# vsergeev/luaradio

Hardware: AMD Instinct MI355X
Metric: MSamples/s per block (128-tap complex FIR headline) + WBFM chain end-to-end (higher is better)
Workload: dtype f32

## Files before the change

luaradio_amd/csrc/kernels_fir.h:

```cpp
#pragma once
#include "common.h"
#include "kernels_elem.h"

#ifndef LRHIP_FIR_PIPE
#define LRHIP_FIR_PIPE 2
#endif
#ifndef LRHIP_DISC_EPI_LDS
#define LRHIP_DISC_EPI_LDS 0
#endif

namespace lrhip {

typedef float f32x4 __attribute__((ext_vector_type(4)));

#ifndef LRHIP_FIR_SETPRIO
#define LRHIP_FIR_SETPRIO 0
#endif
#ifndef LRHIP_FIR_SCHED
#define LRHIP_FIR_SCHED 0
#endif
#ifndef LRHIP_FIR_XCD_MAP
#define LRHIP_FIR_XCD_MAP 0
#endif
#ifndef LRHIP_FIR_WAVES_PER_SIMD
// ... 140 lines not shown
            v1 = o.y;
        } else if (ROT) {
            float2 o = rotate_sample(make_float2(v0, v1), rot_step_fx, rot_count0 + (uint64_t)(p - (M - 1)));
            v0 = o.x;
            v1 = o.y;
        }
        int pa = G::phys(S * r);
        ldsX[pa] = v0;
        if (S == 2) ldsX[pa + 1] = v1;
    }
}

__host__ __device__ constexpr int fir_taps_zl(int D) { return 3 + 15 * D; }
__host__ __device__ constexpr int fir_taps_len(int D, int ksteps) { return ((fir_taps_zl(D) + 4 * ksteps + 3) / 4) * 4; }

template <int S, int D, int NACC, int KS, int NOUT, int TQS = 0>
__device__ __forceinline__ void mfma_tile(const float *ldsT, int tlen, int e, const float *ldsX, int ksteps, f32x4 (&acc)[NOUT][NACC])
{
    using G = FirMfmaGeom<S, D>;
    const int lane = threadIdx.x & 63, wave = threadIdx.x >> 6;
    const int col = lane & 15, kq = lane >> 4;
    const int blk_in_acc = S == 2 ? (col >> 1) : col;
    const int comp = S == 2 ? (col & 1) : 0;
    constexpr int ACC_STRIDE = (G::ROW + G::PAD) * G::BPA;
    const float *bptr = ldsX + (G::ROW + G::PAD) * ((wave * NACC) * G::BPA + blk_in_acc) + S * kq + comp;
    const float *aptr = ldsT + kq * TQS + fir_taps_zl(D) + kq - e - col * D;
#pragma unroll
    for (int o = 0; o < NOUT; o++)
#pragma unroll
        for (int a = 0; a < NACC; a++) acc[o][a] = (f32x4){0.f, 0.f, 0.f, 0.f};
    auto step = [&](const float *ap, const float *bp, int j) {
        float av[NOUT];
#pragma unroll
        for (int o = 0; o < NOUT; o++) av[o] = ap[o * tlen + 4 * j];
#pragma unroll
        for (int a = 0; a < NACC; a++) {
            float bv = bp[a * ACC_STRIDE + j * 4 * S];
#pragma unroll
            for (int o = 0; o < NOUT; o++) acc[o][a] = __builtin_amdgcn_mfma_f32_16x16x4f32(av[o], bv, acc[o][a], 0, 0, 0);
        }
    };
    if constexpr (KS > 0 && (LRHIP_FIR_PIPE == 1 || (LRHIP_FIR_PIPE == 2 && D > 1))) {
        float av[2][NOUT], bv[2][NACC];
        auto fetch = [&](int buf, int s) {
            const int g = s / G::GROUP, j = s % G::GROUP;
            const float *ap = aptr + 4 * g * G::GROUP, *bp = bptr + g * (G::ROW + G::PAD);
#pragma unroll
            for (int o = 0; o < NOUT; o++) av[buf][o] = ap[o * tlen + 4 * j];
#pragma unroll
            for (int a = 0; a < NACC; a++) bv[buf][a] = bp[a * ACC_STRIDE + j * 4 * S];
        };
        fetch(0, 0);
#pragma unroll
        for (int s = 0; s < KS; s++) {
            if (s + 1 < KS) fetch((s + 1) & 1, s + 1);
            __builtin_amdgcn_sched_barrier(0);
#pragma unroll
            for (int a = 0; a < NACC; a++)
#pragma unroll
                for (int o = 0; o < NOUT; o++) acc[o][a] = __builtin_amdgcn_mfma_f32_16x16x4f32(av[s & 1][o], bv[s & 1][a], acc[o][a], 0, 0, 0);
            __builtin_amdgcn_sched_barrier(0);
        }
    } else if constexpr (KS > 0) {
#if LRHIP_FIR_SETPRIO
        __builtin_amdgcn_s_setprio(1);
#endif
#pragma unroll
        for (int g = 0; g < (KS + G::GROUP - 1) / G::GROUP; g++)
#pragma unroll
            for (int j = 0; j < G::GROUP; j++)
// ... 14 lines not shown
}

template <int S, int D, int KS, int TQS, int NR>
__device__ __forceinline__ void mfma_load_areg(const float *ldsT, int e, float (&areg)[NR])
{
    using G = FirMfmaGeom<S, D>;
    const int lane = threadIdx.x & 63;
    const int col = lane & 15, kq = lane >> 4;
    const float *aptr = ldsT + kq * TQS + fir_taps_zl(D) + kq - e - col * D;
#pragma unroll
    for (int s = 0; s < NR; s++) areg[s] = aptr[4 * (s / G::GROUP) * G::GROUP + 4 * (s % G::GROUP)];
}
#ifndef LRHIP_MFMA_AREG_DEPTH
#define LRHIP_MFMA_AREG_DEPTH 1
#endif
template <int S, int D, int NACC, int KS, int TQS, int NR, int SPLIT = 1>
__device__ __forceinline__ void mfma_tile_areg(const float (&areg)[NR], const float *ldsT, int e, const float *ldsX, f32x4 (&acc)[1][NACC])
{
    using G = FirMfmaGeom<S, D>;
    static_assert(NR <= KS, "register-resident steps");
    const int lane = threadIdx.x & 63, wave = threadIdx.x >> 6;
    const int col = lane & 15, kq = lane >> 4;
    const int blk_in_acc = S == 2 ? (col >> 1) : col;
    const int comp = S == 2 ? (col & 1) : 0;
    constexpr int ACC_STRIDE = (G::ROW + G::PAD) * G::BPA;
    const float *bptr = ldsX + (G::ROW + G::PAD) * ((wave * NACC) * G::BPA + blk_in_acc) + S * kq + comp;
    const float *aptr = ldsT + kq * TQS + fir_taps_zl(D) + kq - e - col * D;
    f32x4 acc2[NACC];
#pragma unroll
    for (int a = 0; a < NACC; a++) acc[0][a] = acc2[a] = (f32x4){0.f, 0.f, 0.f, 0.f};
    constexpr int DEPTH = LRHIP_MFMA_AREG_DEPTH, NB = DEPTH + 1;
    float bv[NB][NACC], av[NB];
    auto fetch = [&](int buf, int s) {
        const int g = s / G::GROUP, j = s % G::GROUP;
        const float *bp = bptr + g * (G::ROW + G::PAD);
#pragma unroll
        for (int a = 0; a < NACC; a++) bv[buf][a] = bp[a * ACC_STRIDE + j * 4 * S];
        if (s >= NR) av[buf] = aptr[4 * g * G::GROUP + 4 * j];
    };
#pragma unroll
    for (int s = 0; s < DEPTH && s < KS; s++) fetch(s % NB, s);
#pragma unroll
    for (int s = 0; s < KS; s++) {
        if (s + DEPTH < KS) fetch((s + DEPTH) % NB, s + DEPTH);
        __builtin_amdgcn_sched_barrier(0);
#pragma unroll
        for (int a = 0; a < NACC; a++) {
            const float af = s < NR ? areg[s < NR ? s : 0] : av[s % NB];
            if (SPLIT == 2 && (s & 1)) acc2[a] = __builtin_amdgcn_mfma_f32_16x16x4f32(af, bv[s % NB][a], acc2[a], 0, 0, 0);
            else acc[0][a] = __builtin_amdgcn_mfma_f32_16x16x4f32(af, bv[s % NB][a], acc[0][a], 0, 0, 0);
        }
        __builtin_amdgcn_sched_barrier(0);
    }
    if (SPLIT == 2) {
#pragma unroll
        for (int a = 0; a < NACC; a++) acc[0][a] += acc2[a];
    }
}

// ... 539 lines not shown
            float *o = y + 2 * k;
            if (out_aligned && k + 3 < n_out) {
                *reinterpret_cast<float4 *>(o) = make_float4(dl[0], acc[0][a][0], dl[1], acc[0][a][1]);
                *reinterpret_cast<float4 *>(o + 4) = make_float4(dl[2], acc[0][a][2], dl[3], acc[0][a][3]);
            } else {
#pragma unroll
                for (int i = 0; i < 4; i++)
                    if (k + i < n_out) *reinterpret_cast<float2 *>(o + 2 * i) = make_float2(dl[i], acc[0][a][i]);
            }
        }
    } else {
        store_tile<S, D, NACC, NOUT>(y, tile_k0, n_out, out_aligned, acc);
    }
}

template <int S, int D, int NACC, bool ROT, int KS, int EPI = 0, bool REL = false, int NW = 4, int FMT = 0>
__global__ __launch_bounds__(64 * NW, LRHIP_FIR_WAVES_PER_SIMD) void fir_mfma_persistent_kernel(
    const float *__restrict__ hist, const float *__restrict__ x, const float *__restrict__ taps_pad, float *__restrict__ y,
    int M, long n, long n_out, long first, int e, long ntiles, int out_aligned,
    uint64_t rot_step_fx, uint64_t rot_count0, float2 *__restrict__ edge, float2 *__restrict__ prev_out, double inv_gain, float *__restrict__ hist_out, int rounds)
{
    using G = FirMfmaGeom<S, D>;
    constexpr int NT = 64 * NW;
    static_assert(NW == 4 || (NW == 1 && REL), "one-wave workgroups: relative rotator staging + discriminator epilogue only");
    constexpr int TILE_OUT = G::tile_out(NACC, NW);
    constexpr int SPAN = G::span(NACC, KS, NW);
    static_assert(FMT == 0 || (S == 2 && !REL && EPI == 0 && NW == 4), "raw records: the plain Tuner / Decimator instantiations");
    if (hist_out && blockIdx.x == 0)
        for (int i = threadIdx.x; i < (M - 1) * S; i += NT) hist_out[i] = FMT ? stream_at_raw<FMT>(hist, x, n + i / S, i % S, M, n) : stream_at<S>(hist, x, n + i / S, i % S, M, n);
    constexpr int NF4 = SPAN * S / 4;
    constexpr int UX = (NF4 + NT - 1) / NT;
    extern __shared__ __attribute__((aligned(16))) float lds[];
    constexpr int TLEN = fir_taps_len(D, KS);
    float *ldsT = lds;
    float *ldsX = lds + TLEN;
    const int tid = threadIdx.x;
// ... 50 lines not shown
                const int idx = i4_of(u), ic = idx < 0 ? 0 : idx < NF4 ? idx : NF4 - 1;
                if (FMT == RX_FMT_S16LE) praw[FMT ? u : 0] = reinterpret_cast<const uint2 *>(src0)[ic];
                else praw[FMT ? u : 0].x = reinterpret_cast<const unsigned *>(src0)[ic];
            }
        } else if (have) {
            const float4 *src = reinterpret_cast<const float4 *>(x + xlo_of(tt) * S);
#pragma unroll
            for (int u = 0; u < NPRE; u++) {
                int idx = i4_of(u);
                pre[FMT ? 0 : u] = src[idx < 0 ? 0 : idx < NF4 ? idx : NF4 - 1];
            }
        }
    };
    auto pre_of = [&](int u) -> float4 { if constexpr (FMT != 0) return rx_raw_pair<FMT>(praw[u]); else return pre[u]; };
    prefetch(t);
    for (; t < ntiles; t = tile_of(++tk)) {
        const long tile_k0 = t * (long)TILE_OUT;
        if (have) {
            const long xlo = xlo_of(t);
            if constexpr (REL) {
#pragma unroll
                for (int u = 0; u < UX; u++) {
                    const int i4 = tid + u * NT;
                    const cf a = cmul(cf{pre[u].x, pre[u].y}, rel_w[u][0]), b = cmul(cf{pre[u].z, pre[u].w}, rel_w[u][1]);
                    if (i4 < NF4) lds_put4<S, D>(ldsX, i4, make_float4(a.x, a.y, b.x, b.y));
                }
            } else if constexpr (ROT) {
#pragma unroll
                for (int v = 0; v < UB; v++) {
                    const int i40 = 4 * (tid + NT * v) - a4;
// ... 9 lines not shown
                        if (i40 + 2 >= 0 && i40 + 2 < NF4) lds_put4<S, D>(ldsX, i40 + 2, rotate_in_block<2>(pre_of(4 * v + 2), p, rot_t));
                        if (i40 + 3 < NF4) lds_put4<S, D>(ldsX, i40 + 3, rotate_in_block<3>(pre_of(4 * v + 3), p, rot_t));
                    }
                }
            } else {
#pragma unroll
                for (int u = 0; u < UX; u++) {
                    const int i4 = tid + u * NT;
                    if (i4 < NF4) lds_put4<S, D>(ldsX, i4, pre_of(u));
                }
            }
        } else {
            stage_edge<S, D, ROT, REL, NT, FMT>(ldsX, hist, x, first + tile_k0 * D - e, SPAN, M, n, rot_step_fx, rot_count0);
        }
        __syncthreads();
        prefetch(tile_of(tk + 1));
        f32x4 acc[1][NACC];
        mfma_tile<S, D, NACC, KS, 1>(ldsT, TLEN, e, ldsX, KS, acc);
        if constexpr (EPI == 0) {
            store_tile<S, D, NACC, 1>(y, tile_k0, n_out, out_aligned, acc);
        } else {
            static_assert(S == 2, "discriminator epilogue: complex stream");
#if LRHIP_DISC_EPI_LDS
            disc_epilogue_lds<D, NACC>(y, ldsX, tile_k0, n_out, acc, edge + 2 * t, prev_out, inv_gain);
#else
            cf pt = cf{1.f, 0.f};
            if constexpr (REL) pt = phasor_poly(rot_step_fx * (rot_count0 + (uint64_t)xlo_of(t)));
            const bool stream_start = REL && t == 0 && rot_count0 == 0 && first == 0 && n > 0;
            float2 o_first = make_float2(0.f, 0.f);
            if constexpr (REL) {
                if (stream_start) {
                    const float h0 = ldsT[fir_taps_zl(D) + M - 1];
                    const float2 x0 = rotate_sample(*reinterpret_cast<const float2 *>(x), rot_step_fx, (uint64_t)0);
                    o_first = make_float2(fmaf(h0, x0.x, 0.f), fmaf(h0, x0.y, 0.f));
                }
            }
            disc_epilogue<D, NACC, REL>(y, tile_k0, n_out, out_aligned, acc, edge + 2 * NW * t, prev_out, inv_gain, pt, stream_start, o_first);
#endif
        }
        __syncthreads();
    }
}

inline int fir_mfma_ksteps(int M, int D, int S, int emax_override = -1)
{
    int emax = emax_override >= 0 ? emax_override : 4 / S - 1;
    return (emax + 15 * D + M + 3) / 4;
}
inline void fir_mfma_build_taps(const float *taps_rev, int M, int D, int ksteps, std::vector<float> &out)
{
    out.assign((size_t)fir_taps_len(D, ksteps), 0.f);
    for (int j = 0; j < M; j++) out[(size_t)fir_taps_zl(D) + j] = taps_rev[j];
}

}
```

luaradio_amd/csrc/kernels_rx.h:

```cpp
#pragma once
#include "kernels_fir.h"

#ifndef LRHIP_RX_AREG
#define LRHIP_RX_AREG 40
#endif
#ifndef LRHIP_RX_SPLITK
#define LRHIP_RX_SPLITK 1
#endif

namespace lrhip {

struct RxParams {
    const float *hist;
    const float *x;
    long n;
    const float *taps_pad;
    long n_out_a, first_a;
    int e;
    long ntiles;
    uint64_t rot_step_fx, rot_count0;
    const float2 *prev_in;
    float2 *prev_out;
    double inv_gain;
    float *hist_out;
// ... 70 lines not shown
    const uint8_t *b = reinterpret_cast<const uint8_t *>(x) + 2 * xi;
    return rx_raw_sample<FMT>(b[0], b[1]);
}

#ifdef LRHIP_RX_TRACE
__device__ unsigned long long *lrhip_rx_trace;
#define RX_STAMP(i)                                                                                                                                 \
    do {                                                                                                                                            \
        if (lrhip_rx_trace && blockIdx.x < 8 && trace_tile < 64 && (threadIdx.x & 63) == 0)                                                         \
            lrhip_rx_trace[(((size_t)blockIdx.x * 4 + (threadIdx.x >> 6)) * 64 + trace_tile) * 8 + (i)] = clock64();                                  \
    } while (0)
#else
#define RX_STAMP(i) do { } while (0)
#endif

template <int FMT>
__global__ __launch_bounds__(256, LRHIP_RX_WAVES_PER_SIMD) void rx_fused_kernel(const RxParams pr)
{
    constexpr bool U8 = FMT != RX_FMT_CF32;
    constexpr int NT = 256, D = RX_D, S = 2, M = RX_M;
    constexpr int NF4 = RX_SPAN * S / 4;
    constexpr int UX = (NF4 + NT - 1) / NT;
    static_assert(2 * UX <= 64, "one lane per uniform phasor");
    extern __shared__ __attribute__((aligned(16))) float lds[];
    float *ldsT = lds, *ldsX = lds + RX_LDS_X, *P = lds + RX_LDS_P, *ldsGT = lds + RX_LDS_G, *ldsPt = lds + RX_LDS_PT, *xch = lds + RX_LDS_XCH;
    float2 *eo = reinterpret_cast<float2 *>(lds + RX_LDS_EO);
    const int tid = threadIdx.x, lane = tid & 63, wave = tid >> 6;
    const long n = pr.n;
    const float *__restrict__ x = pr.x;
    const float *__restrict__ hist = pr.hist;

    if (pr.hist_out && blockIdx.x == 0)
        for (int i = tid; i < M - 1; i += NT) {
            const cf v = rx_stream_at<FMT>(hist, x, n + i, M, n);
            pr.hist_out[2 * i] = v.x;
            pr.hist_out[2 * i + 1] = v.y;
        }
    for (int i = tid; i < RX_TLEN; i += NT) {
// ... 28 lines not shown
    auto xlo_of = [&](long tt) { return pr.first_a + tt * (long)RX_TILE * D - pr.e - (M - 1); };
    auto interior = [&](long tt) { const long lo = xlo_of(tt); return tt < tend && lo >= 0 && lo + RX_SPAN <= n; };

    cf rel_w[UX][2];
    {
        const cf pt = phasor_poly(pr.rot_step_fx * (uint64_t)(2 * tid)), pu = phasor_poly(pr.rot_step_fx * (uint64_t)(2 * NT * (lane >> 1) + (lane & 1)));
#pragma unroll
        for (int u = 0; u < UX; u++)
#pragma unroll
            for (int j = 0; j < 2; j++) rel_w[u][j] = cmul(pt, cf{__shfl(pu.x, 2 * u + j), __shfl(pu.y, 2 * u + j)});
    }

    float4 pre[U8 ? 1 : UX];
    uint2 pre8[U8 ? UX : 1];
    bool have = false;
    auto prefetch = [&](long tt) {
        have = interior(tt);
        if (U8) {
            if (have) {
                const uint8_t *src0 = reinterpret_cast<const uint8_t *>(x) + 2 * rx_raw_bytes<FMT>() * xlo_of(tt);
#pragma unroll
                for (int u = 0; u < UX; u++) {
                    const int idx = tid + NT * u, ic = idx < NF4 ? idx : NF4 - 1;
                    if (FMT == RX_FMT_S16LE) pre8[u] = reinterpret_cast<const uint2 *>(src0)[ic];
                    else pre8[u].x = reinterpret_cast<const unsigned *>(src0)[ic];
                }
            }
        } else if (have && (pr.dbg & 8)) {
#pragma unroll
            for (int u = 0; u < UX; u++) pre[u] = make_float4(0.5f, 0.25f, -0.5f, 0.125f);
        } else if (have) {
            const float4 *src = reinterpret_cast<const float4 *>(x + xlo_of(tt) * S);
#pragma unroll
            for (int u = 0; u < UX; u++) {
                const int idx = tid + NT * u;
                pre[u] = src[idx < NF4 ? idx : NF4 - 1];
            }
        }
    };
    prefetch(t);

    [[maybe_unused]] int trace_tile = 0;
    for (; t < tend; t++) {
        RX_STAMP(0);
        const bool warm = t < t0;
        const int tau = warm ? RX_TPB - 1 : (int)((t - t0) % RX_TPB);
        const long bidx = warm ? 0 : (t - t0) / RX_TPB;
        const long tile_k0 = t * (long)RX_TILE;
        if (have) {
#pragma unroll
            for (int u = 0; u < UX; u++) {
                const int i4 = tid + u * NT;
                cf s0, s1;
                if (U8) {
                    if (FMT == RX_FMT_S16LE) {
                        s0 = rx_raw_sample<FMT>(pre8[u].x & 0xffffu, pre8[u].x >> 16);
                        s1 = rx_raw_sample<FMT>(pre8[u].y & 0xffffu, pre8[u].y >> 16);
// ... 12 lines not shown
        } else if (U8) {
            using GE = FirMfmaGeom<S, D>;
            const long base = pr.first_a + tile_k0 * D - pr.e;
            for (int r = tid; r < RX_SPAN; r += NT) {
                const cf o = cmul(rx_stream_at<FMT>(hist, x, base + r, M, n), rel_window_phasor<NT>(pr.rot_step_fx, r));
                const int pa = GE::phys(S * r);
                ldsX[pa] = o.x;
                ldsX[pa + 1] = o.y;
            }
        } else {
            stage_edge<S, D, true, true, NT>(ldsX, hist, x, pr.first_a + tile_k0 * D - pr.e, RX_SPAN, M, n, pr.rot_step_fx, pr.rot_count0);
        }
        RX_STAMP(1);
        __syncthreads();
        RX_STAMP(2);
        prefetch(t + 1 < tend ? t + 1 : tend);
        RX_STAMP(3);

        f32x4 acc[1][RX_NACC];
        if (pr.dbg & 4) {
#pragma unroll
            for (int a = 0; a < RX_NACC; a++) acc[0][a] = (f32x4){ldsX[tid], ldsX[tid + 256], ldsX[tid + 512], ldsX[tid + 768]};
        }
#if LRHIP_RX_AREG
        else mfma_tile_areg<S, D, RX_NACC, RX_KS, RX_TQS, LRHIP_RX_AREG, LRHIP_RX_SPLITK>(areg, ldsT, pr.e, ldsX, acc);
#else
        else mfma_tile<S, D, RX_NACC, RX_KS, 1, RX_TQS>(ldsT, RX_TLEN, pr.e, ldsX, RX_KS, acc);
#endif

        RX_STAMP(4);
#if LRHIP_RX_NACC == 1
        {
            const int col = lane & 15, kq = lane >> 4;
            const bool odd = col & 1;
            const int src = odd ? lane - 1 : kq ? lane - 15 : col ? col + 47 : 63;
            const float a0 = acc[0][0][0], a1 = acc[0][0][1], a2 = acc[0][0][2], a3 = acc[0][0][3];
            const float recv0 = __shfl_xor(odd ? a0 : a2, 1);
            const float recv1 = __shfl_xor(odd ? a1 : a3, 1);
            const float2 o0 = odd ? make_float2(recv0, a2) : make_float2(a0, recv0);
            const float2 o1 = odd ? make_float2(recv1, a3) : make_float2(a1, recv1);
            float2 p = make_float2(__shfl(o1.x, src), __shfl(o1.y, src));
            float2 *eo_t = eo + 4 * (int)(t & 1), *eo_p = eo + 4 * (int)((t & 1) ^ 1);
            if (lane == 63) eo_t[wave] = o1;
// ... 65 lines not shown
        RX_STAMP(7);
#ifdef LRHIP_RX_TRACE
        trace_tile++;
#endif
        const bool last_tile = t == pr.ntiles - 1;
        if (tau == RX_TPB - 1 || t == tend - 1) {
            __syncthreads();
            f32x4 acct[1][1];
            acct[0][0] = (f32x4){0.f, 0.f, 0.f, 0.f};
            if (!(pr.dbg & 1) && wave < RX_AW && (!warm || wave == RX_AW - 1)) mfma_tile<1, D, 1, RX_KST, 1>(ldsGT + RX_GZ, RX_GLEN - RX_GZ, phi, P, RX_KST, acct);
            float *vrow = ldsX;
            {
                const int col = lane & 15, kq = lane >> 4;
                if (wave < RX_AW) *reinterpret_cast<float4 *>(vrow + 16 * (wave * 16 + col) + 4 * kq) = make_float4(acct[0][0][0], acct[0][0][1], acct[0][0][2], acct[0][0][3]);
            }
            __syncthreads();
            const bool scan_lane = tid < 64 * RX_AW;
            float4 v4 = scan_lane ? *reinterpret_cast<const float4 *>(vrow + 4 * tid) : make_float4(0.f, 0.f, 0.f, 0.f);
            if (warm) {
                const int kmin = (RX_TH + (RX_TPB - 1) * RX_TILE + 1 - phi + 4) / 5;
                const int k = 4 * tid;
                v4 = make_float4(k >= kmin ? v4.x : 0.f, k + 1 >= kmin ? v4.y : 0.f, k + 2 >= kmin ? v4.z : 0.f, k + 3 >= kmin ? v4.w : 0.f);
            }
            const float u0 = pr.b0 * v4.x, u1 = pr.b0 * v4.y, u2 = pr.b0 * v4.z, u3 = pr.b0 * v4.w;
            auto stepq = [&](float stv, float uv) { return fmaf(pr.na1, stv, fmaf(pr.na1_lo, stv, uv)); };
            float z = stepq(stepq(stepq(u0, u1), u2), u3);
#pragma unroll
            for (int l = 0; l < 6; l++) {
                const float prev = __shfl_up(z, 1 << l);
                if (lane >= (1 << l)) z = z + fmaf(ldsPt[(1 << l) - 1], prev, 0.f);
            }
// ... 26 lines not shown
                if (!ends_with_batch && last >= 0 && last < 4) pr.state_out[0] = last == 0 ? y0 : last == 1 ? y1 : last == 2 ? y2 : y3;
                if (ends_with_batch && tid == 0) pr.state_out[0] = C;
            }
            carry = C;
            __syncthreads();
            if (last_tile) {
                const int ev = (int)(pr.n_out_a - (t0 * RX_TILE + bidx * RX_BATCH));
                if (tid < RX_TH) pr.thist_out[tid] = P[rx_pos(ev - RX_TH + tid)];
            } else if (tid < RX_TH) {
                P[rx_pos(tid - RX_TH)] = P[rx_pos(RX_BATCH - RX_TH + tid)];
            }
        }
    }
}

}
```

luaradio_amd/csrc/stage_fir.h:

```cpp
#pragma once
#include "fir_form.h"

struct FirStage : lrhip_stage, FirShape {
    FirStage() { rel_rot = !LRHIP_DISC_EPI_LDS && getenv("LRHIP_TUNER_EXACT") == nullptr;
                 rel_nw1 = getenv("LRHIP_TUNER_NW1") != nullptr; }
    std::vector<float> taps_rev;
    std::vector<float> natural_taps() const
    {
        const int ts = taps_complex ? 2 : 1;
        std::vector<float> h((size_t)M * ts);
        for (int t = 0; t < M; t++)
            for (int c = 0; c < ts; c++) h[(size_t)t * ts + c] = taps_rev[(size_t)(M - 1 - t) * ts + c];
        return h;
    }
    DeviceBuf d_taps, d_atab, d_ctaps4;
    int mfma_blocks_per_cu = 0;
    int hist_pad = 0;
    DeviceBuf hist[2];
    int cur = 0;
    unsigned long index = 0;
    uint64_t rot_step = 0, count = 0;
    long L = 0, fill = 0;
    DeviceBuf pending, work;
    static constexpr int FFT_PART = FIR_FFT_PART;
// ... 108 lines not shown
        const unsigned esz = raw_now ? (in_fmt == RX_FMT_S16LE ? 4u : 2u) : (unsigned)(4 * SS);
        if (((uintptr_t)x % esz) != 0) return set_error("fir: fused rotator / discriminator needs a sample-aligned input pointer");
        long sample_addr = (long)((uintptr_t)x / esz);
        int q = 4 / SS;
        long v = sample_addr + (long)index - (M - 1);
        int e = (int)(((v % q) + q) % q);
        int span = G::span(NACC, ksteps, NW);
        size_t lds_floats = (size_t)fir_taps_len(DD, ksteps) + (size_t)G::phys(SS * span) + G::PAD + 8;
        size_t lds_bytes = lds_floats * sizeof(float);
        long ntiles = (n_out + TILE_OUT - 1) / TILE_OUT;
        const float *atab = (const float *)d_atab.p;
        const float *h = (const float *)hist[cur].p + hist_pad;
        int out_aligned = ((uintptr_t)y % 16) == 0;
        uint64_t rs = rot ? rot_step : 0, rc = rot ? count : 0;
        if constexpr (KS > 0) {
            auto launch = [&](auto kern) -> int {
                if ((mfma_blocks_per_cu = prepared_blocks(kern, lds_bytes, 64 * NW)) < 0) return -1;
                long slots = (long)ctx().num_cus * mfma_blocks_per_cu;
                const int rounds = ntiles > slots && fir_knobs().fir_rounds > 0 ? fir_knobs().fir_rounds : 0;
                unsigned grid = rounds > 0 ? (unsigned)((ntiles + rounds - 1) / rounds) : (unsigned)(ntiles < slots ? ntiles : slots);
                if (post_disc && edge.reserve((size_t)ntiles * 2 * NW * sizeof(float2))) return -1;
                float *ho = M > 1 ? (float *)hist[cur ^ 1].p + hist_pad : nullptr;
                hipLaunchKernelGGL(kern, dim3(grid), dim3(64 * NW), lds_bytes, ctx().stream, h, x, atab, y, M, n, n_out, (long)index, e,
                                   ntiles, out_aligned, rs, rc, (float2 *)edge.p, post_disc ? (float2 *)disc_prev.p + (disc_cur ^ 1) : nullptr, 1.0 / disc_gain, ho, rounds);
                hist_in_kernel = ho != nullptr;
                return 0;
            };
            int rc2;
            if constexpr (SS == 2 && (DD == 4 || DD == 8 || DD == 10)) {
                if (!(post_disc && rot)) return set_error("internal: decimation %d has a persistent kernel for tuner + discriminator only", DD);
            }
            if constexpr (SS == 2 && (DD == 1 || DD == 5 || DD == 4 || DD == 8 || DD == 10)) {
                if (post_disc) {
                    if constexpr (DD == 4 || DD == 8 || DD == 10)
                        rc2 = rel_rot ? launch(fir_mfma_persistent_kernel<2, DD, NACC, true, KS, 1, true>) : launch(fir_mfma_persistent_kernel<2, DD, NACC, true, KS, 1, false>);
                    else if constexpr (NW == 1) rc2 = launch(fir_mfma_persistent_kernel<2, DD, NACC, true, KS, 1, true, 1>);
                    else if constexpr (LRHIP_DISC_EPI_LDS) rc2 = rot ? launch(fir_mfma_persistent_kernel<2, DD, NACC, true, KS, 1>) : launch(fir_mfma_persistent_kernel<2, DD, NACC, false, KS, 1>);
                    else rc2 = !rot ? launch(fir_mfma_persistent_kernel<2, DD, NACC, false, KS, 1>)
                             : rel_rot ? launch(fir_mfma_persistent_kernel<2, DD, NACC, true, KS, 1, true>) : launch(fir_mfma_persistent_kernel<2, DD, NACC, true, KS, 1, false>);
                    if (rc2) return rc2;
                    LR_LAUNCH_CHECK();
                    float2 *dp = (float2 *)disc_prev.p;
                    constexpr int FIX_UNIT = LRHIP_DISC_EPI_LDS ? TILE_OUT : TILE_OUT / NW;
                    const long nunits = LRHIP_DISC_EPI_LDS ? ntiles : NW * ntiles;
                    if (defer_fixup && (FIX_UNIT & (FIX_UNIT - 1)) == 0 && FIX_UNIT >= 256) {
                        fix_ready = true;
                        fix_nunits = nunits; fix_unit = FIX_UNIT;
                        fix_prev_ptr = (const float2 *)(dp + disc_cur);
                        fix_shift = 0;
                        while ((1 << fix_shift) < FIX_UNIT) fix_shift++;
                    } else {
                        hipLaunchKernelGGL(fir_disc_fixup_kernel, dim3((unsigned)((nunits + 255) / 256)), dim3(256), 0, ctx().stream, (const float2 *)edge.p,
                                           nunits, FIX_UNIT, y, n_out, (const float2 *)(dp + disc_cur), 1.0 / disc_gain);
                        LR_LAUNCH_CHECK();
                    }
                    disc_cur ^= 1;
                    return 0;
                }
            }
            if (post_disc) return set_error("internal: discriminator epilogue without a persistent kernel variant");
            if constexpr (SS == 2 && DD == 5 && KS == 51 && NW == 4) {
                if (raw_now) {
                    if (rot)
                        rc2 = in_fmt == RX_FMT_U8 ? launch(fir_mfma_persistent_kernel<2, DD, NACC, true, KS, 0, false, 4, RX_FMT_U8>)
                            : in_fmt == RX_FMT_S8 ? launch(fir_mfma_persistent_kernel<2, DD, NACC, true, KS, 0, false, 4, RX_FMT_S8>)
                                                  : launch(fir_mfma_persistent_kernel<2, DD, NACC, true, KS, 0, false, 4, RX_FMT_S16LE>);
                    else
                        rc2 = in_fmt == RX_FMT_U8 ? launch(fir_mfma_persistent_kernel<2, DD, NACC, false, KS, 0, false, 4, RX_FMT_U8>)
                            : in_fmt == RX_FMT_S8 ? launch(fir_mfma_persistent_kernel<2, DD, NACC, false, KS, 0, false, 4, RX_FMT_S8>)
                                                  : launch(fir_mfma_persistent_kernel<2, DD, NACC, false, KS, 0, false, 4, RX_FMT_S16LE>);
                    if (rc2) return rc2;
                    LR_LAUNCH_CHECK();
                    return 0;
                }
            }
            if (raw_now) return set_error("internal: raw records reached a kernel without a record instantiation");
            if constexpr (DD == 4 || DD == 8 || DD == 10) return set_error("internal: no plain persistent kernel at decimation %d", DD);
            else {
                if constexpr (SS == 2) rc2 = rot ? launch(fir_mfma_persistent_kernel<2, DD, NACC, true, KS>) : launch(fir_mfma_persistent_kernel<2, DD, NACC, false, KS>);
                else rc2 = rot ? set_error("rotator fusion needs complex input") : launch(fir_mfma_persistent_kernel<1, DD, NACC, false, KS>);
                if (rc2) return rc2;
            }
        } else {
            if (post_disc) return set_error("internal: discriminator epilogue without a persistent kernel variant");
            auto launch = [&](auto kern) -> int {
                if (prepare_kernel(kern, lds_bytes, nullptr)) return -1;
                hipLaunchKernelGGL(kern, dim3((unsigned)ntiles), dim3(256), lds_bytes, ctx().stream, h, x, atab, y, M, n, n_out, (long)index, e,
                                   ksteps, out_aligned, rs, rc);
                return 0;
            };
            int rc2;
            if constexpr (SS == 2) rc2 = rot ? launch(fir_mfma_kernel<2, DD, NACC, true, 1>) : launch(fir_mfma_kernel<2, DD, NACC, false, 1>);
            else rc2 = rot ? set_error("rotator fusion needs complex input") : launch(fir_mfma_kernel<1, DD, NACC, false, 1>);
            if (rc2) return rc2;
        }
// ... 921 lines not shown
```

luaradio_amd/csrc/stage_rx.h:

```cpp
#pragma once

struct RxStage : lrhip_stage {
    std::unique_ptr<FirStage> A, B;
    DeviceBuf mid;
    DeviceBuf d_ptab4;
    int blocks_per_cu = 0, blocks_per_cu8 = 0;
    int in_fmt = RX_FMT_CF32;
    bool in_u8 = false;
    lrhip_stage *fmt = nullptr;
    DeviceBuf converted;
    bool single_launch = true;
    int last_form = 0;

    const char *kind() const override { return "fm-receiver"; }
    bool direct_io_ok() const override { return true; }
    unsigned long max_output(unsigned long n) const override { return B->max_output(A->max_output(n)); }
    int reset() override { return (A->reset() || B->reset()) ? -1 : 0; }
    int seek(unsigned long long n0, unsigned long long *n0_out) override
    {
        unsigned long long m = 0;
        if (A->seek(n0, &m) || B->seek(m, n0_out)) return -1;
        return 0;
    }
    long memory() const override
// ... 59 lines not shown
            if (m < 0) return m;
            return run_cf32(converted.p, n_in, out_dev, cap, one, n_out_a, n_out_b, false);
        }
        return run_cf32(in_dev, n_in, out_dev, cap, one, n_out_a, n_out_b, in_u8);
    }

    long run_cf32(const void *in_dev, unsigned long n_in, void *out_dev, unsigned long cap, bool one, long n_out_a, long n_out_b, bool u8)
    {
        const long n = (long)n_in;
        if (!one || (!u8 && ((uintptr_t)in_dev % 8) != 0)) return run_two(in_dev, n_in, out_dev, cap);
        if ((unsigned long)n_out_b > cap) return set_error("fm-receiver: output capacity %lu < %ld", cap, n_out_b);
        const float *x = (const float *)in_dev;
        const size_t lds_bytes = (size_t)RX_LDS_FLOATS * sizeof(float);
        int &bpc = u8 ? blocks_per_cu8 : blocks_per_cu;
        const int fmt_k = u8 ? in_fmt : RX_FMT_CF32;
        auto with_kernel = [&](auto fn) -> int {
            switch (fmt_k) {
                case RX_FMT_U8: return fn(rx_fused_kernel<RX_FMT_U8>);
                case RX_FMT_S8: return fn(rx_fused_kernel<RX_FMT_S8>);
                case RX_FMT_S16LE: return fn(rx_fused_kernel<RX_FMT_S16LE>);
                default: return fn(rx_fused_kernel<RX_FMT_CF32>);
            }
        };
        if (!bpc) {
            const int rc0 = with_kernel([&](auto kern) -> int {
                LR_HIP(hipFuncSetAttribute((const void *)kern, hipFuncAttributeMaxDynamicSharedMemorySize, (int)lds_bytes));
                int nb = 0;
                LR_HIP(hipOccupancyMaxActiveBlocksPerMultiprocessor(&nb, kern, 256, lds_bytes));
                bpc = nb < 1 ? 1 : nb;
                return 0;
            });
            if (rc0) return rc0;
        }
        RxParams pr;
        memset(&pr, 0, sizeof(pr));
        pr.hist = (const float *)A->hist[A->cur].p; pr.x = x; pr.n = n; pr.taps_pad = (const float *)A->d_atab.p;
        pr.n_out_a = n_out_a; pr.first_a = (long)A->index;
        const long v = (long)((uintptr_t)x / (u8 ? (in_fmt == RX_FMT_S16LE ? 4 : 2) : 8)) + (long)A->index - (RX_M - 1);
        pr.e = (int)(((v % 2) + 2) % 2);
        pr.ntiles = (n_out_a + RX_TILE - 1) / RX_TILE;
// ... 12 lines not shown
        if (env_wgs > 0) wgs = (long)ctx().num_cus * env_wgs;
        const long most = (pr.ntiles + 7) / 8;
        if (wgs < 1 || wgs > most) wgs = most;
        pr.dbg = ablation_bits("LRHIP_RX_DBG");
        const unsigned grid = (unsigned)wgs;
#ifdef LRHIP_RX_TRACE
        static unsigned long long *trace = nullptr;
        static long trace_launches = 0;
        const size_t trace_n = (size_t)8 * 4 * 64 * 8;
        if (!trace) {
            LR_HIP(hipMalloc(&trace, trace_n * 8));
            LR_HIP(hipMemcpyToSymbol(HIP_SYMBOL(lrhip_rx_trace), &trace, sizeof(trace)));
        }
        if (++trace_launches == 12) LR_HIP(hipMemsetAsync(trace, 0, trace_n * 8, ctx().stream));
#endif
        (void)with_kernel([&](auto kern) -> int { hipLaunchKernelGGL(kern, dim3(grid), dim3(256), lds_bytes, ctx().stream, pr); return 0; });
        LR_LAUNCH_CHECK();
#ifdef LRHIP_RX_TRACE
        if (trace_launches == 12) {
            LR_HIP(hipStreamSynchronize(ctx().stream));
            std::vector<unsigned long long> tr(trace_n);
            LR_HIP(hipMemcpy(tr.data(), trace, trace_n * 8, hipMemcpyDeviceToHost));
            static const char *names[8] = {"stage", "barrierA", "prefetch", "mfma", "exchange", "barrierB", "disc", "tail"};
            for (int w = 0; w < 4; w++) {
                double sum[8] = {0, 0, 0, 0, 0, 0, 0, 0}, tile = 0;
                int cnt = 0;
                for (int b = 0; b < 8; b++)
                    for (int t = 2; t < 62; t++) {
                        const unsigned long long *s = &tr[(((size_t)b * 4 + w) * 64 + t) * 8], *nx = s + 8;
                        if (!s[0] || !s[7] || !nx[0]) continue;
                        for (int i = 0; i < 7; i++) sum[i] += (double)(s[i + 1] - s[i]);
// ... 23 lines not shown
```

Measured before the change: 315,500.

## Spread next-tile global prefetch across MFMA steps via hook in pipelined loop

Instead of issuing all next-tile input prefetch loads in one burst before the MFMA tile loop, the loads are spread across the k-steps of the software-pipelined MFMA loop through a per-step hook. They use wave-uniform base pointers with clamped per-lane offsets so addresses are always in bounds. The goal is to overlap global memory traffic with matrix math and smooth out issue pressure. Burst-kernel variants are kept for short inputs and debug modes, which doubles the kernel instantiations. An optional wave-level fence can replace one __syncthreads in the audio path, but only behind a macro.

Result: no change. 315,100 (-0.2%).

```diff
diff --git a/luaradio_amd/csrc/kernels_fir.h b/luaradio_amd/csrc/kernels_fir.h
--- a/luaradio_amd/csrc/kernels_fir.h
+++ b/luaradio_amd/csrc/kernels_fir.h
@@ -1,4 +1,5 @@
 #pragma once
+#include <type_traits>
 #include "common.h"
 #include "kernels_elem.h"
 
@@ -178,9 +179,47 @@
 __host__ __device__ constexpr int fir_taps_zl(int D) { return 3 + 15 * D; }
 __host__ __device__ constexpr int fir_taps_len(int D, int ksteps) { return ((fir_taps_zl(D) + 4 * ksteps + 3) / 4) * 4; }
 
-template <int S, int D, int NACC, int KS, int NOUT, int TQS = 0>
-__device__ __forceinline__ void mfma_tile(const float *ldsT, int tlen, int e, const float *ldsX, int ksteps, f32x4 (&acc)[NOUT][NACC])
-{
+struct MfmaNoHook {
+    __device__ __forceinline__ void operator()(int) const {}
+};
+template <int KS, int NLOAD>
+__host__ __device__ constexpr int spread_first(int s)
+{
+    static_assert(KS > 2 && NLOAD > 0, "spread prefetch: steps to spread over");
+    const int u = s < 2 ? 0 : ((s - 2) * NLOAD + KS - 3) / (KS - 2);
+    return u < NLOAD ? u : NLOAD;
+}
+template <int KS, int NLOAD>
+constexpr int SPREAD_PER_STEP = (NLOAD + KS - 3) / (KS - 2);
+typedef const __attribute__((address_space(1))) char *wave_uniform_ptr;
+__device__ __forceinline__ wave_uniform_ptr wave_uniform(const void *p)
+{
+    const uint64_t v = reinterpret_cast<uint64_t>(p);
+    const uint32_t lo = __builtin_amdgcn_readfirstlane((uint32_t)v), hi = __builtin_amdgcn_readfirstlane((uint32_t)(v >> 32));
+    return (wave_uniform_ptr)(((uint64_t)hi << 32) | lo);
+}
+template <class T>
+__device__ __forceinline__ T wave_uniform_load(wave_uniform_ptr p)
+{
+    if constexpr (std::is_same<T, float4>::value) {
+        const f32x4 v = *(const __attribute__((address_space(1))) f32x4 *)p;
+        return make_float4(v[0], v[1], v[2], v[3]);
+    } else if constexpr (std::is_same<T, uint2>::value) {
+        typedef unsigned u32x2 __attribute__((ext_vector_type(2)));
+        const u32x2 v = *(const __attribute__((address_space(1))) u32x2 *)p;
+        return make_uint2(v[0], v[1]);
+    } else {
+        return *(const __attribute__((address_space(1))) T *)p;
+    }
+}
+__host__ __device__ constexpr int fir_spread_align(int S, int FMT) { return FMT ? 2 : 4 / S; }
+__host__ __device__ constexpr long fir_spread_min_samples(int span, int S, int FMT) { return (long)span + fir_spread_align(S, FMT) - 1; }
+__host__ __device__ constexpr bool mfma_tile_piped(int KS, int D) { return KS > 0 && (LRHIP_FIR_PIPE == 1 || (LRHIP_FIR_PIPE == 2 && D > 1)); }
+
+template <int S, int D, int NACC, int KS, int NOUT, int TQS = 0, class HOOK = MfmaNoHook>
+__device__ __forceinline__ void mfma_tile(const float *ldsT, int tlen, int e, const float *ldsX, int ksteps, f32x4 (&acc)[NOUT][NACC], HOOK hook = HOOK{})
+{
+    static_assert(mfma_tile_piped(KS, D) || std::is_same<HOOK, MfmaNoHook>::value, "only the software-pipelined loop calls the hook");
     using G = FirMfmaGeom<S, D>;
     const int lane = threadIdx.x & 63, wave = threadIdx.x >> 6;
     const int col = lane & 15, kq = lane >> 4;
@@ -204,7 +243,7 @@
             for (int o = 0; o < NOUT; o++) acc[o][a] = __builtin_amdgcn_mfma_f32_16x16x4f32(av[o], bv, acc[o][a], 0, 0, 0);
         }
     };
-    if constexpr (KS > 0 && (LRHIP_FIR_PIPE == 1 || (LRHIP_FIR_PIPE == 2 && D > 1))) {
+    if constexpr (mfma_tile_piped(KS, D)) {
         float av[2][NOUT], bv[2][NACC];
         auto fetch = [&](int buf, int s) {
             const int g = s / G::GROUP, j = s % G::GROUP;
@@ -218,6 +257,7 @@
 #pragma unroll
         for (int s = 0; s < KS; s++) {
             if (s + 1 < KS) fetch((s + 1) & 1, s + 1);
+            hook(s);
             __builtin_amdgcn_sched_barrier(0);
 #pragma unroll
             for (int a = 0; a < NACC; a++)
@@ -262,8 +302,8 @@
 #ifndef LRHIP_MFMA_AREG_DEPTH
 #define LRHIP_MFMA_AREG_DEPTH 1
 #endif
-template <int S, int D, int NACC, int KS, int TQS, int NR, int SPLIT = 1>
-__device__ __forceinline__ void mfma_tile_areg(const float (&areg)[NR], const float *ldsT, int e, const float *ldsX, f32x4 (&acc)[1][NACC])
+template <int S, int D, int NACC, int KS, int TQS, int NR, int SPLIT = 1, class HOOK = MfmaNoHook>
+__device__ __forceinline__ void mfma_tile_areg(const float (&areg)[NR], const float *ldsT, int e, const float *ldsX, f32x4 (&acc)[1][NACC], HOOK hook = HOOK{})
 {
     using G = FirMfmaGeom<S, D>;
     static_assert(NR <= KS, "register-resident steps");
@@ -291,6 +331,7 @@
 #pragma unroll
     for (int s = 0; s < KS; s++) {
         if (s + DEPTH < KS) fetch((s + DEPTH) % NB, s + DEPTH);
+        hook(s);
         __builtin_amdgcn_sched_barrier(0);
 #pragma unroll
         for (int a = 0; a < NACC; a++) {
@@ -860,12 +901,13 @@
     }
 }
 
-template <int S, int D, int NACC, bool ROT, int KS, int EPI = 0, bool REL = false, int NW = 4, int FMT = 0>
-__global__ __launch_bounds__(64 * NW, LRHIP_FIR_WAVES_PER_SIMD) void fir_mfma_persistent_kernel(
+template <bool SPREAD, int S, int D, int NACC, bool ROT, int KS, int EPI, bool REL, int NW, int FMT>
+__device__ __forceinline__ void fir_mfma_persistent_body(
     const float *__restrict__ hist, const float *__restrict__ x, const float *__restrict__ taps_pad, float *__restrict__ y,
     int M, long n, long n_out, long first, int e, long ntiles, int out_aligned,
     uint64_t rot_step_fx, uint64_t rot_count0, float2 *__restrict__ edge, float2 *__restrict__ prev_out, double inv_gain, float *__restrict__ hist_out, int rounds)
 {
+    static_assert(!SPREAD || mfma_tile_piped(KS, D), "spread prefetch: the loop with the hook");
     using G = FirMfmaGeom<S, D>;
     constexpr int NT = 64 * NW;
     static_assert(NW == 4 || (NW == 1 && REL), "one-wave workgroups: relative rotator staging + discriminator epilogue only");
@@ -946,6 +988,23 @@
     };
     auto pre_of = [&](int u) -> float4 { if constexpr (FMT != 0) return rx_raw_pair<FMT>(praw[u]); else return pre[u]; };
     prefetch(t);
+    auto window_at = [&](long xlo) -> const char * {
+        return reinterpret_cast<const char *>(x) + (FMT != 0 ? 2 * rx_raw_bytes<FMT>() : 4 * S) * xlo;
+    };
+    auto load_pre = [&](const char *src, int u) {
+        constexpr int LM = ROT && !REL ? 4 : 1, EB = FMT == 0 ? 16 : FMT == RX_FMT_S16LE ? 8 : 4;
+        const int cu = ROT && !REL ? 4 * NT * (u >> 2) + (u & 3) - a4 : NT * u, c = cu < NF4 - 1 ? cu : NF4 - 1;
+        const int l = LM * tid + (cu - c), lc = l < -c ? -c : l > NF4 - 1 - c ? NF4 - 1 - c : l;
+        unsigned off = EB * lc;
+        asm volatile("" : "+v"(off));
+        wave_uniform_ptr p = wave_uniform(src + (long)EB * c) + off;
+        if constexpr (FMT == RX_FMT_S16LE) praw[u] = wave_uniform_load<uint2>(p);
+        else if constexpr (FMT != 0) praw[u].x = wave_uniform_load<unsigned>(p);
+        else pre[u] = wave_uniform_load<float4>(p);
+    };
+    constexpr int QA = fir_spread_align(S, FMT);
+    static_assert((TILE_OUT * D) % QA == 0, "every window has the alignment of the first");
+    const long xlo_fb = ((xlo_of(0) % QA) + QA) % QA;
     for (; t < ntiles; t = tile_of(++tk)) {
         const long tile_k0 = t * (long)TILE_OUT;
         if (have) {
@@ -985,9 +1044,23 @@
             stage_edge<S, D, ROT, REL, NT, FMT>(ldsX, hist, x, first + tile_k0 * D - e, SPAN, M, n, rot_step_fx, rot_count0);
         }
         __syncthreads();
-        prefetch(tile_of(tk + 1));
         f32x4 acc[1][NACC];
-        mfma_tile<S, D, NACC, KS, 1>(ldsT, TLEN, e, ldsX, KS, acc);
+        if constexpr (SPREAD) {
+            const long tn = tile_of(tk + 1);
+            const bool have_next = interior(tn);
+            const char *src = window_at(have_next ? xlo_of(tn) : xlo_fb);
+            mfma_tile<S, D, NACC, KS, 1>(ldsT, TLEN, e, ldsX, KS, acc, [&](int s) {
+#pragma unroll
+                for (int j = 0; j < SPREAD_PER_STEP<KS, NPRE>; j++) {
+                    const int u = spread_first<KS, NPRE>(s) + j;
+                    if (u < spread_first<KS, NPRE>(s + 1)) load_pre(src, u);
+                }
+            });
+            have = have_next;
+        } else {
+            prefetch(tile_of(tk + 1));
+            mfma_tile<S, D, NACC, KS, 1>(ldsT, TLEN, e, ldsX, KS, acc);
+        }
         if constexpr (EPI == 0) {
             store_tile<S, D, NACC, 1>(y, tile_k0, n_out, out_aligned, acc);
         } else {
@@ -1013,6 +1086,29 @@
     }
 }
 
+#define LRHIP_FIR_PERSISTENT_ARGS                                                                                                                        \
+    const float *__restrict__ hist, const float *__restrict__ x, const float *__restrict__ taps_pad, float *__restrict__ y, int M, long n, long n_out, \
+        long first, int e, long ntiles, int out_aligned, uint64_t rot_step_fx, uint64_t rot_count0, float2 *__restrict__ edge,                          \
+        float2 *__restrict__ prev_out, double inv_gain, float *__restrict__ hist_out, int rounds
+#define LRHIP_FIR_PERSISTENT_PASS hist, x, taps_pad, y, M, n, n_out, first, e, ntiles, out_aligned, rot_step_fx, rot_count0, edge, prev_out, inv_gain, hist_out, rounds
+template <int S, int D, int NACC, bool ROT, int KS, int EPI = 0, bool REL = false, int NW = 4, int FMT = 0>
+__global__ __launch_bounds__(64 * NW, LRHIP_FIR_WAVES_PER_SIMD) void fir_mfma_persistent_kernel(LRHIP_FIR_PERSISTENT_ARGS)
+{
+    fir_mfma_persistent_body<mfma_tile_piped(KS, D), S, D, NACC, ROT, KS, EPI, REL, NW, FMT>(LRHIP_FIR_PERSISTENT_PASS);
+}
+template <int S, int D, int NACC, bool ROT, int KS, int EPI = 0, bool REL = false, int NW = 4, int FMT = 0>
+__global__ __launch_bounds__(64 * NW, LRHIP_FIR_WAVES_PER_SIMD) void fir_mfma_persistent_burst_kernel(LRHIP_FIR_PERSISTENT_ARGS)
+{
+    fir_mfma_persistent_body<false, S, D, NACC, ROT, KS, EPI, REL, NW, FMT>(LRHIP_FIR_PERSISTENT_PASS);
+}
+template <auto... A>
+struct FirPersistent {
+    static constexpr auto kernel() { return &fir_mfma_persistent_kernel<A...>; }
+    static constexpr auto burst_kernel() { return &fir_mfma_persistent_burst_kernel<A...>; }
+};
+#undef LRHIP_FIR_PERSISTENT_ARGS
+#undef LRHIP_FIR_PERSISTENT_PASS
+
 inline int fir_mfma_ksteps(int M, int D, int S, int emax_override = -1)
 {
     int emax = emax_override >= 0 ? emax_override : 4 / S - 1;
diff --git a/luaradio_amd/csrc/kernels_rx.h b/luaradio_amd/csrc/kernels_rx.h
--- a/luaradio_amd/csrc/kernels_rx.h
+++ b/luaradio_amd/csrc/kernels_rx.h
@@ -108,14 +108,15 @@
 #define RX_STAMP(i) do { } while (0)
 #endif
 
-template <int FMT>
-__global__ __launch_bounds__(256, LRHIP_RX_WAVES_PER_SIMD) void rx_fused_kernel(const RxParams pr)
+template <int FMT, bool SPREAD>
+__device__ __forceinline__ void rx_fused_body(const RxParams &pr)
 {
     constexpr bool U8 = FMT != RX_FMT_CF32;
     constexpr int NT = 256, D = RX_D, S = 2, M = RX_M;
     constexpr int NF4 = RX_SPAN * S / 4;
     constexpr int UX = (NF4 + NT - 1) / NT;
     static_assert(2 * UX <= 64, "one lane per uniform phasor");
+    static_assert(fir_spread_align(S, FMT) == 2, "window alignment: two samples");
     extern __shared__ __attribute__((aligned(16))) float lds[];
     float *ldsT = lds, *ldsX = lds + RX_LDS_X, *P = lds + RX_LDS_P, *ldsGT = lds + RX_LDS_G, *ldsPt = lds + RX_LDS_PT, *xch = lds + RX_LDS_XCH;
     float2 *eo = reinterpret_cast<float2 *>(lds + RX_LDS_EO);
@@ -174,6 +175,19 @@
     float4 pre[U8 ? 1 : UX];
     uint2 pre8[U8 ? UX : 1];
     bool have = false;
+    auto window_at = [&](long xlo) -> const char * {
+        return reinterpret_cast<const char *>(x) + (U8 ? 2 * rx_raw_bytes<FMT>() : 4 * S) * xlo;
+    };
+    auto load_pre = [&](const char *src, int u) {
+        constexpr int EB = !U8 ? 16 : FMT == RX_FMT_S16LE ? 8 : 4;
+        const int c = NT * u, lc = tid > NF4 - 1 - c ? NF4 - 1 - c : tid;
+        unsigned off = EB * lc;
+        asm volatile("" : "+v"(off));
+        wave_uniform_ptr p = wave_uniform(src + (long)EB * c) + off;
+        if constexpr (FMT == RX_FMT_S16LE) pre8[u] = wave_uniform_load<uint2>(p);
+        else if constexpr (U8) pre8[u].x = wave_uniform_load<unsigned>(p);
+        else pre[u] = wave_uniform_load<float4>(p);
+    };
     auto prefetch = [&](long tt) {
         have = interior(tt);
         if (U8) {
@@ -201,6 +215,7 @@
     prefetch(t);
 
     [[maybe_unused]] int trace_tile = 0;
+    const long xlo_fb = ((xlo_of(0) % 2) + 2) % 2;
     for (; t < tend; t++) {
         RX_STAMP(0);
         const bool warm = t < t0;
@@ -243,19 +258,32 @@
         RX_STAMP(1);
         __syncthreads();
         RX_STAMP(2);
-        prefetch(t + 1 < tend ? t + 1 : tend);
+        const long tn = t + 1 < tend ? t + 1 : tend;
+        const bool have_next = interior(tn);
+        [[maybe_unused]] const char *src = window_at(have_next ? xlo_of(tn) : xlo_fb);
+        [[maybe_unused]] auto spread = [&](int s) {
+#pragma unroll
+            for (int j = 0; j < SPREAD_PER_STEP<RX_KS, UX>; j++) {
+                const int u = spread_first<RX_KS, UX>(s) + j;
+                if (u < spread_first<RX_KS, UX>(s + 1)) load_pre(src, u);
+            }
+        };
+        if constexpr (!SPREAD) prefetch(tn);
         RX_STAMP(3);
 
         f32x4 acc[1][RX_NACC];
-        if (pr.dbg & 4) {
+        if (!SPREAD && (pr.dbg & 4)) {
 #pragma unroll
             for (int a = 0; a < RX_NACC; a++) acc[0][a] = (f32x4){ldsX[tid], ldsX[tid + 256], ldsX[tid + 512], ldsX[tid + 768]};
         }
 #if LRHIP_RX_AREG
+        else if constexpr (SPREAD) mfma_tile_areg<S, D, RX_NACC, RX_KS, RX_TQS, LRHIP_RX_AREG, LRHIP_RX_SPLITK>(areg, ldsT, pr.e, ldsX, acc, spread);
         else mfma_tile_areg<S, D, RX_NACC, RX_KS, RX_TQS, LRHIP_RX_AREG, LRHIP_RX_SPLITK>(areg, ldsT, pr.e, ldsX, acc);
 #else
+        else if constexpr (SPREAD) mfma_tile<S, D, RX_NACC, RX_KS, 1, RX_TQS>(ldsT, RX_TLEN, pr.e, ldsX, RX_KS, acc, spread);
         else mfma_tile<S, D, RX_NACC, RX_KS, 1, RX_TQS>(ldsT, RX_TLEN, pr.e, ldsX, RX_KS, acc);
 #endif
+        if constexpr (SPREAD) have = have_next;
 
         RX_STAMP(4);
 #if LRHIP_RX_NACC == 1
@@ -351,7 +379,13 @@
                 const int col = lane & 15, kq = lane >> 4;
                 if (wave < RX_AW) *reinterpret_cast<float4 *>(vrow + 16 * (wave * 16 + col) + 4 * kq) = make_float4(acct[0][0][0], acct[0][0][1], acct[0][0][2], acct[0][0][3]);
             }
-            __syncthreads();
+#ifdef LRHIP_RX_AUDIO_WAVEFENCE
+            __builtin_amdgcn_fence(__ATOMIC_RELEASE, "wavefront");
+            __builtin_amdgcn_wave_barrier();
+            __builtin_amdgcn_fence(__ATOMIC_ACQUIRE, "wavefront");
+#else
+            __syncthreads();
+#endif
             const bool scan_lane = tid < 64 * RX_AW;
             float4 v4 = scan_lane ? *reinterpret_cast<const float4 *>(vrow + 4 * tid) : make_float4(0.f, 0.f, 0.f, 0.f);
             if (warm) {
@@ -408,4 +442,15 @@
     }
 }
 
+template <int FMT>
+__global__ __launch_bounds__(256, LRHIP_RX_WAVES_PER_SIMD) void rx_fused_kernel(const RxParams pr)
+{
+    rx_fused_body<FMT, true>(pr);
 }
+template <int FMT>
+__global__ __launch_bounds__(256, LRHIP_RX_WAVES_PER_SIMD) void rx_fused_burst_kernel(const RxParams pr)
+{
+    rx_fused_body<FMT, false>(pr);
+}
+
+}
diff --git a/luaradio_amd/csrc/stage_fir.h b/luaradio_amd/csrc/stage_fir.h
--- a/luaradio_amd/csrc/stage_fir.h
+++ b/luaradio_amd/csrc/stage_fir.h
@@ -146,7 +146,12 @@
         int out_aligned = ((uintptr_t)y % 16) == 0;
         uint64_t rs = rot ? rot_step : 0, rc = rot ? count : 0;
         if constexpr (KS > 0) {
-            auto launch = [&](auto kern) -> int {
+            const bool burst = mfma_tile_piped(KS, DD) && n < fir_spread_min_samples(span, SS, raw_now ? in_fmt : 0);
+            auto launch = [&](auto pair) -> int {
+                auto kern = pair.kernel();
+                if constexpr (mfma_tile_piped(KS, DD)) {
+                    if (burst) kern = pair.burst_kernel();
+                }
                 if ((mfma_blocks_per_cu = prepared_blocks(kern, lds_bytes, 64 * NW)) < 0) return -1;
                 long slots = (long)ctx().num_cus * mfma_blocks_per_cu;
                 const int rounds = ntiles > slots && fir_knobs().fir_rounds > 0 ? fir_knobs().fir_rounds : 0;
@@ -165,11 +170,11 @@
             if constexpr (SS == 2 && (DD == 1 || DD == 5 || DD == 4 || DD == 8 || DD == 10)) {
                 if (post_disc) {
                     if constexpr (DD == 4 || DD == 8 || DD == 10)
-                        rc2 = rel_rot ? launch(fir_mfma_persistent_kernel<2, DD, NACC, true, KS, 1, true>) : launch(fir_mfma_persistent_kernel<2, DD, NACC, true, KS, 1, false>);
-                    else if constexpr (NW == 1) rc2 = launch(fir_mfma_persistent_kernel<2, DD, NACC, true, KS, 1, true, 1>);
-                    else if constexpr (LRHIP_DISC_EPI_LDS) rc2 = rot ? launch(fir_mfma_persistent_kernel<2, DD, NACC, true, KS, 1>) : launch(fir_mfma_persistent_kernel<2, DD, NACC, false, KS, 1>);
-                    else rc2 = !rot ? launch(fir_mfma_persistent_kernel<2, DD, NACC, false, KS, 1>)
-                             : rel_rot ? launch(fir_mfma_persistent_kernel<2, DD, NACC, true, KS, 1, true>) : launch(fir_mfma_persistent_kernel<2, DD, NACC, true, KS, 1, false>);
+                        rc2 = rel_rot ? launch(FirPersistent<2, DD, NACC, true, KS, 1, true>{}) : launch(FirPersistent<2, DD, NACC, true, KS, 1, false>{});
+                    else if constexpr (NW == 1) rc2 = launch(FirPersistent<2, DD, NACC, true, KS, 1, true, 1>{});
+                    else if constexpr (LRHIP_DISC_EPI_LDS) rc2 = rot ? launch(FirPersistent<2, DD, NACC, true, KS, 1>{}) : launch(FirPersistent<2, DD, NACC, false, KS, 1>{});
+                    else rc2 = !rot ? launch(FirPersistent<2, DD, NACC, false, KS, 1>{})
+                             : rel_rot ? launch(FirPersistent<2, DD, NACC, true, KS, 1, true>{}) : launch(FirPersistent<2, DD, NACC, true, KS, 1, false>{});
                     if (rc2) return rc2;
                     LR_LAUNCH_CHECK();
                     float2 *dp = (float2 *)disc_prev.p;
@@ -194,13 +199,13 @@
             if constexpr (SS == 2 && DD == 5 && KS == 51 && NW == 4) {
                 if (raw_now) {
                     if (rot)
-                        rc2 = in_fmt == RX_FMT_U8 ? launch(fir_mfma_persistent_kernel<2, DD, NACC, true, KS, 0, false, 4, RX_FMT_U8>)
-                            : in_fmt == RX_FMT_S8 ? launch(fir_mfma_persistent_kernel<2, DD, NACC, true, KS, 0, false, 4, RX_FMT_S8>)
-                                                  : launch(fir_mfma_persistent_kernel<2, DD, NACC, true, KS, 0, false, 4, RX_FMT_S16LE>);
+                        rc2 = in_fmt == RX_FMT_U8 ? launch(FirPersistent<2, DD, NACC, true, KS, 0, false, 4, RX_FMT_U8>{})
+                            : in_fmt == RX_FMT_S8 ? launch(FirPersistent<2, DD, NACC, true, KS, 0, false, 4, RX_FMT_S8>{})
+                                                  : launch(FirPersistent<2, DD, NACC, true, KS, 0, false, 4, RX_FMT_S16LE>{});
                     else
-                        rc2 = in_fmt == RX_FMT_U8 ? launch(fir_mfma_persistent_kernel<2, DD, NACC, false, KS, 0, false, 4, RX_FMT_U8>)
-                            : in_fmt == RX_FMT_S8 ? launch(fir_mfma_persistent_kernel<2, DD, NACC, false, KS, 0, false, 4, RX_FMT_S8>)
-                                                  : launch(fir_mfma_persistent_kernel<2, DD, NACC, false, KS, 0, false, 4, RX_FMT_S16LE>);
+                        rc2 = in_fmt == RX_FMT_U8 ? launch(FirPersistent<2, DD, NACC, false, KS, 0, false, 4, RX_FMT_U8>{})
+                            : in_fmt == RX_FMT_S8 ? launch(FirPersistent<2, DD, NACC, false, KS, 0, false, 4, RX_FMT_S8>{})
+                                                  : launch(FirPersistent<2, DD, NACC, false, KS, 0, false, 4, RX_FMT_S16LE>{});
                     if (rc2) return rc2;
                     LR_LAUNCH_CHECK();
                     return 0;
@@ -209,8 +214,8 @@
             if (raw_now) return set_error("internal: raw records reached a kernel without a record instantiation");
             if constexpr (DD == 4 || DD == 8 || DD == 10) return set_error("internal: no plain persistent kernel at decimation %d", DD);
             else {
-                if constexpr (SS == 2) rc2 = rot ? launch(fir_mfma_persistent_kernel<2, DD, NACC, true, KS>) : launch(fir_mfma_persistent_kernel<2, DD, NACC, false, KS>);
-                else rc2 = rot ? set_error("rotator fusion needs complex input") : launch(fir_mfma_persistent_kernel<1, DD, NACC, false, KS>);
+                if constexpr (SS == 2) rc2 = rot ? launch(FirPersistent<2, DD, NACC, true, KS>{}) : launch(FirPersistent<2, DD, NACC, false, KS>{});
+                else rc2 = rot ? set_error("rotator fusion needs complex input") : launch(FirPersistent<1, DD, NACC, false, KS>{});
                 if (rc2) return rc2;
             }
         } else {
diff --git a/luaradio_amd/csrc/stage_rx.h b/luaradio_amd/csrc/stage_rx.h
--- a/luaradio_amd/csrc/stage_rx.h
+++ b/luaradio_amd/csrc/stage_rx.h
@@ -97,16 +97,21 @@
         const size_t lds_bytes = (size_t)RX_LDS_FLOATS * sizeof(float);
         int &bpc = u8 ? blocks_per_cu8 : blocks_per_cu;
         const int fmt_k = u8 ? in_fmt : RX_FMT_CF32;
-        auto with_kernel = [&](auto fn) -> int {
+        auto with_kernel = [&](bool burst, auto fn) -> int {
             switch (fmt_k) {
-                case RX_FMT_U8: return fn(rx_fused_kernel<RX_FMT_U8>);
-                case RX_FMT_S8: return fn(rx_fused_kernel<RX_FMT_S8>);
-                case RX_FMT_S16LE: return fn(rx_fused_kernel<RX_FMT_S16LE>);
-                default: return fn(rx_fused_kernel<RX_FMT_CF32>);
+                case RX_FMT_U8: return burst ? fn(rx_fused_burst_kernel<RX_FMT_U8>) : fn(rx_fused_kernel<RX_FMT_U8>);
+                case RX_FMT_S8: return burst ? fn(rx_fused_burst_kernel<RX_FMT_S8>) : fn(rx_fused_kernel<RX_FMT_S8>);
+                case RX_FMT_S16LE: return burst ? fn(rx_fused_burst_kernel<RX_FMT_S16LE>) : fn(rx_fused_kernel<RX_FMT_S16LE>);
+                default: return burst ? fn(rx_fused_burst_kernel<RX_FMT_CF32>) : fn(rx_fused_kernel<RX_FMT_CF32>);
             }
         };
         if (!bpc) {
-            const int rc0 = with_kernel([&](auto kern) -> int {
+            const int rc1 = with_kernel(true, [&](auto kern) -> int {
+                LR_HIP(hipFuncSetAttribute((const void *)kern, hipFuncAttributeMaxDynamicSharedMemorySize, (int)lds_bytes));
+                return 0;
+            });
+            if (rc1) return rc1;
+            const int rc0 = with_kernel(false, [&](auto kern) -> int {
                 LR_HIP(hipFuncSetAttribute((const void *)kern, hipFuncAttributeMaxDynamicSharedMemorySize, (int)lds_bytes));
                 int nb = 0;
                 LR_HIP(hipOccupancyMaxActiveBlocksPerMultiprocessor(&nb, kern, 256, lds_bytes));
@@ -149,7 +154,8 @@
         }
         if (++trace_launches == 12) LR_HIP(hipMemsetAsync(trace, 0, trace_n * 8, ctx().stream));
 #endif
-        (void)with_kernel([&](auto kern) -> int { hipLaunchKernelGGL(kern, dim3(grid), dim3(256), lds_bytes, ctx().stream, pr); return 0; });
+        const bool burst = n < fir_spread_min_samples(RX_SPAN, 2, fmt_k) || (pr.dbg & 12) != 0;
+        (void)with_kernel(burst, [&](auto kern) -> int { hipLaunchKernelGGL(kern, dim3(grid), dim3(256), lds_bytes, ctx().stream, pr); return 0; });
         LR_LAUNCH_CHECK();
 #ifdef LRHIP_RX_TRACE
         if (trace_launches == 12) {
```
